# DefTruth/CUDA-Learn-Notes

Measured on NVIDIA H100. Metric: hgemm_tflops, higher is better.
Workload: dtype f16 (fp32 accumulate)

## Files before the change

### cuda-learn-notes_b200/csrc/hgemm_wgmma.cu

```cuda
#include "abi_common.cuh"
#include "ptx.cuh"

namespace b200k {

namespace gemm {
constexpr int BM = 128, BN = 256, STAGES = 4, THREADS = 384, GROUP_M = 16;
constexpr int STG_BYTES = 16384;
}

template <int DT_, bool A_MN_, bool B_MN_>
struct GemmCfg {
  static constexpr int DT = DT_;
  static constexpr bool A_MN = A_MN_, B_MN = B_MN_;
  static constexpr int ES = DT == 2 ? 4 : 2;
  static constexpr int BK = 128 / ES;
  static constexpr int KSTEP = DT == 2 ? 8 : 16;
  static constexpr int A_BYTES = gemm::BM * BK * ES;
  static constexpr int B_BYTES = gemm::BN * BK * ES;
  static constexpr int STAGE_BYTES = A_BYTES + B_BYTES;
  static constexpr int SMEM_BYTES = gemm::STAGES * STAGE_BYTES + 2 * gemm::STG_BYTES + 1024 + 2 * gemm::STAGES * 8;
  static_assert(!(DT == 2 && (A_MN || B_MN)), "tf32 wgmma reads K-major operands only");
  static_assert(SMEM_BYTES <= 232448, "more shared memory than an H100 block may use");
};

template <class Cfg>
__device__ __forceinline__ void gemm_mma_kblock(float* d, uint32_t sA, uint32_t sB, int cw) {
  constexpr int STEPS = Cfg::BK / Cfg::KSTEP;
#pragma unroll
  for (int k = 0; k < STEPS; ++k) {
    const uint64_t da = Cfg::A_MN ? wgmma_desc(sA + cw * 64 * Cfg::BK * Cfg::ES + k * 2048, 64 * Cfg::BK * Cfg::ES, 1024)
                                  : wgmma_desc(sA + cw * 64 * 128 + k * 32, 16, 1024);
    const uint64_t db = Cfg::B_MN ? wgmma_desc(sB + k * 2048, 64 * Cfg::BK * Cfg::ES, 1024) : wgmma_desc(sB + k * 32, 16, 1024);
    wgmma_ss<Cfg::DT, 256, Cfg::A_MN, Cfg::B_MN>(d, da, db, 1);
  }
}

template <class Cfg>
__device__ __forceinline__ void gemm_store_tile(const float* d, const CUtensorMap* tmC, uint32_t stg, int cw, int row0,
                                                int col0) {
  constexpr int SLICES = Cfg::DT == 2 ? 4 : 2, JS = 32 / SLICES, JB = JS / 2;
  const int t = threadIdx.x & 127, lane = t & 31, warp = t / 32;
  const bool leader = t == 0;
#pragma unroll
  for (int sl = 0; sl < SLICES; ++sl) {
    if (leader) tma_store_wait_read<0>();
    named_bar_sync(1 + cw, 128);
    if constexpr (Cfg::DT == 2) {
      const int q = lane & 3;
#pragma unroll
      for (int jj = 0; jj < JS; ++jj) {
        const int j = sl * JS + jj;
#pragma unroll
        for (int h = 0; h < 2; ++h) {
          const int r = warp * 16 + 8 * h + lane / 4;
          const int chunk = 2 * (jj % JB) + q / 2;
          const uint32_t a = stg + (jj / JB) * 8192 + r * 128 + ((chunk ^ (r & 7)) << 4) + (q & 1) * 8;
          asm volatile("st.shared.v2.f32 [%0], {%1, %2};" ::"r"(a), "f"(d[4 * j + 2 * h]), "f"(d[4 * j + 2 * h + 1])
                       : "memory");
        }
      }
    } else {
      const int m = lane / 8, r = warp * 16 + 8 * (m & 1) + (lane & 7);
#pragma unroll
      for (int jj = 0; jj < JS; jj += 2) {
        const int j = sl * JS + jj, chunk = jj % JB + (m >> 1);
        const uint32_t a = stg + (jj / JB) * 8192 + r * 128 + ((chunk ^ (r & 7)) << 4);
        uint32_t p[4];
#pragma unroll
        for (int i = 0; i < 4; ++i)
          p[i] = Cfg::DT == 1 ? pack_bf162(d[4 * j + 2 * i], d[4 * j + 2 * i + 1])
                              : pack_half2(d[4 * j + 2 * i], d[4 * j + 2 * i + 1]);
        stmatrix_x4(a, p[0], p[1], p[2], p[3]);
      }
    }
    fence_proxy_async_smem();
    named_bar_sync(1 + cw, 128);
    if (leader) {
      const int c = col0 + sl * (gemm::BN / SLICES);
      tma_store_2d(tmC, stg, c, row0);
      tma_store_2d(tmC, stg + 8192, c + 128 / Cfg::ES, row0);
      tma_store_commit();
    }
  }
}

template <class Cfg>
__global__ void __launch_bounds__(gemm::THREADS, 1)
    hgemm_wgmma_kernel(const __grid_constant__ CUtensorMap tmA, const __grid_constant__ CUtensorMap tmB,
                       const __grid_constant__ CUtensorMap tmC, int K, int tiles_m, int tiles_n) {
  using namespace gemm;
  extern __shared__ uint8_t smem_raw[];
  const uint32_t base = (smem_u32(smem_raw) + 1023) & ~1023u;
  const uint32_t stg0 = base + STAGES * Cfg::STAGE_BYTES;
  const uint32_t full0 = stg0 + 2 * STG_BYTES, empty0 = full0 + STAGES * 8;
  const int wg = threadIdx.x / 128;

  const int tile = blockIdx.x, width = GROUP_M * tiles_n, g = tile / width, first_m = g * GROUP_M;
  const int gsz = min(tiles_m - first_m, GROUP_M);
  const int tm = first_m + (tile % width) % gsz, tn = (tile % width) / gsz;
  const int nkb = (K + Cfg::BK - 1) / Cfg::BK;

  if (threadIdx.x == 0) {
    for (int s = 0; s < STAGES; ++s) {
      mbar_init(full0 + 8 * s, 1);
      mbar_init(empty0 + 8 * s, 2);
    }
    fence_mbar_init();
  }
  __syncthreads();

  if (wg == 0) {
    if (threadIdx.x == 0) {
      tma_prefetch_desc(&tmA);
      tma_prefetch_desc(&tmB);
      for (int kb = 0; kb < nkb; ++kb) {
        const int s = kb % STAGES;
        if (kb >= STAGES) mbar_wait_nocall(empty0 + 8 * s, ((kb / STAGES) - 1) & 1);
        const uint32_t bar = full0 + 8 * s, sA = base + s * Cfg::STAGE_BYTES, sB = sA + Cfg::A_BYTES;
        mbar_arrive_expect_tx(bar, Cfg::STAGE_BYTES);
        if constexpr (Cfg::A_MN) {
#pragma unroll
          for (int c = 0; c < BM / 64; ++c)
            tma_load_2d(sA + c * 64 * Cfg::BK * Cfg::ES, &tmA, bar, tm * BM + c * 64, kb * Cfg::BK, kPolicyEvictNormal);
        } else {
          tma_load_2d(sA, &tmA, bar, kb * Cfg::BK, tm * BM, kPolicyEvictNormal);
        }
        if constexpr (Cfg::B_MN) {
#pragma unroll
          for (int c = 0; c < BN / 64; ++c)
            tma_load_2d(sB + c * 64 * Cfg::BK * Cfg::ES, &tmB, bar, tn * BN + c * 64, kb * Cfg::BK, kPolicyEvictNormal);
        } else {
          tma_load_2d(sB, &tmB, bar, kb * Cfg::BK, tn * BN, kPolicyEvictNormal);
        }
      }
    }
    return;
  }

  const int cw = wg - 1, t = threadIdx.x & 127;
  const bool leader = t == 0;
  if (leader) tma_prefetch_desc(&tmC);
  float d[128];
#pragma unroll
  for (int i = 0; i < 128; ++i) d[i] = 0.f;
  for (int kb = 0; kb < nkb; ++kb) {
    const int s = kb % STAGES;
    mbar_wait_nocall(full0 + 8 * s, (kb / STAGES) & 1);
    const uint32_t sA = base + s * Cfg::STAGE_BYTES, sB = sA + Cfg::A_BYTES;
    fence_regs<128>(d);
    wgmma_fence();
    gemm_mma_kblock<Cfg>(d, sA, sB, cw);
    wgmma_commit();
    wgmma_wait<1>();
    fence_regs<128>(d);
    if (kb > 0 && leader) mbar_arrive(empty0 + 8 * ((kb - 1) % STAGES));
  }
  wgmma_wait<0>();
  fence_regs<128>(d);
  gemm_store_tile<Cfg>(d, &tmC, stg0 + cw * STG_BYTES, cw, tm * BM + cw * 64, tn * BN);
  if (leader) tma_store_wait_all<0>();
}

template <class Cfg>
static int launch_gemm(const void* A, const void* B, void* C, int64_t M, int64_t N, int64_t K, cudaStream_t s,
                       const DeviceInfo& di) {
  using namespace gemm;
  auto tmap = [](CUtensorMap* m, const void* p, int64_t rows, int64_t cols, uint32_t box_rows, uint32_t box_cols) {
    const uint64_t dims[2] = {uint64_t(cols), uint64_t(rows)}, strides[1] = {uint64_t(cols) * Cfg::ES};
    const uint32_t box[2] = {box_cols, box_rows};
    return make_tmap(m, p, Cfg::ES, 2, dims, strides, box);
  };
  CUtensorMap tmA, tmB, tmC;
  int rc = Cfg::A_MN ? tmap(&tmA, A, K, M, Cfg::BK, 64) : tmap(&tmA, A, M, K, BM, Cfg::BK);
  if (rc) return rc;
  rc = Cfg::B_MN ? tmap(&tmB, B, K, N, Cfg::BK, 64) : tmap(&tmB, B, N, K, BN, Cfg::BK);
  if (rc) return rc;
  if ((rc = tmap(&tmC, C, M, N, 64, 128 / Cfg::ES))) return rc;
  const int64_t tiles_m = (M + BM - 1) / BM, tiles_n = (N + BN - 1) / BN, tiles = tiles_m * tiles_n;
  if (tiles > INT32_MAX) return set_error(B200K_ESHAPE, "GEMM too large: %lld tiles", (long long)tiles);
  auto kern = hgemm_wgmma_kernel<Cfg>;
  if ((rc = ensure_dynamic_smem(reinterpret_cast<const void*>(kern), di.device, Cfg::SMEM_BYTES))) return rc;
  kern<<<unsigned(tiles), THREADS, Cfg::SMEM_BYTES, s>>>(tmA, tmB, tmC, int(K), int(tiles_m), int(tiles_n));
  B200K_CHECK_CUDA(cudaGetLastError());
  return B200K_OK;
}

template <int DT>
static int gemm_dispatch(const char* who, const void* A, const void* B, void* C, int64_t M, int64_t N, int64_t K,
                         int b_is_nk, int variant, void* stream, int a_is_km = 0) {
  constexpr int PACK = (DT == 2) ? 4 : 8;
  if (!A || !B || !C) return set_error(B200K_EARG, "%s: null pointer", who);
  if (reinterpret_cast<uintptr_t>(C) & 15) return set_error(B200K_EALIGN, "%s: C (%p) must be 16-byte aligned", who, C);
  if (M < 1 || N < 1 || K < 1 || M > INT32_MAX || N > INT32_MAX || K > INT32_MAX)
    return set_error(B200K_ESHAPE, "%s: M,N,K must be in [1, 2^31) (got %lld,%lld,%lld)", who, (long long)M, (long long)N,
                     (long long)K);
  if ((K % PACK) || (N % PACK))
    return set_error(B200K_ESHAPE, "%s: K and N must be multiples of %d (16-byte rows), got K=%lld N=%lld", who, PACK,
                     (long long)K, (long long)N);
  if (a_is_km && DT == 2) return set_error(B200K_EDTYPE, "%s: A stored as [K,M] is built for f16 / bf16 only", who);
  if (a_is_km && (M % PACK))
    return set_error(B200K_ESHAPE, "%s: M must be a multiple of %d when A is stored as [K,M]", who, PACK);
  const int v = variant & 0xff;
  if (v < B200K_HGEMM_AUTO || v > B200K_HGEMM_2CTA_512x256)
    return set_error(B200K_EARG, "%s: variant %d unknown", who, v);
  DeviceInfo di;
  int rc = get_device_info(&di);
  if (rc) return rc;
  cudaStream_t s = static_cast<cudaStream_t>(stream);
  const bool nn = (b_is_nk == 0);
  if constexpr (DT == 2) {
    if (!nn) return launch_gemm<GemmCfg<2, false, false>>(A, B, C, M, N, K, s, di);
    void* bt = nullptr;
    B200K_CHECK_CUDA(cudaMallocAsync(&bt, size_t(K) * size_t(N) * 4, s));
    rc = b200k_mat_transpose_f32(B, bt, K, N, stream);
    if (!rc) rc = launch_gemm<GemmCfg<2, false, false>>(A, bt, C, M, N, K, s, di);
    cudaError_t e = cudaFreeAsync(bt, s);
    if (!rc && e != cudaSuccess) rc = set_error(B200K_ECUDA, "cudaFreeAsync failed: %s", cudaGetErrorString(e));
    return rc;
  } else {
    if (a_is_km)
      return nn ? launch_gemm<GemmCfg<DT, true, true>>(A, B, C, M, N, K, s, di)
                : launch_gemm<GemmCfg<DT, true, false>>(A, B, C, M, N, K, s, di);
    return nn ? launch_gemm<GemmCfg<DT, false, true>>(A, B, C, M, N, K, s, di)
              : launch_gemm<GemmCfg<DT, false, false>>(A, B, C, M, N, K, s, di);
  }
}

}

extern "C" int b200k_hgemm_f16(const void* A, const void* B, void* C, int64_t M, int64_t N, int64_t K, int b_is_nk,
                               int variant, void* stream) {
  return b200k::gemm_dispatch<0>("b200k_hgemm_f16", A, B, C, M, N, K, b_is_nk, variant, stream);
}

extern "C" int b200k_gemm_ex(const void* A, const void* B, void* C, int64_t M, int64_t N, int64_t K, int a_is_km, int b_is_nk,
                             int dtype, int variant, void* stream) {
  switch (dtype) {
    case B200K_F16: return b200k::gemm_dispatch<0>("b200k_gemm_ex(f16)", A, B, C, M, N, K, b_is_nk, variant, stream, a_is_km);
    case B200K_BF16: return b200k::gemm_dispatch<1>("b200k_gemm_ex(bf16)", A, B, C, M, N, K, b_is_nk, variant, stream, a_is_km);
    case B200K_F32: return b200k::gemm_dispatch<2>("b200k_gemm_ex(tf32)", A, B, C, M, N, K, b_is_nk, variant, stream, a_is_km);
    default: return b200k::set_error(B200K_EDTYPE, "b200k_gemm_ex: dtype %d not supported (f16, bf16, f32-as-tf32)", dtype);
  }
}

extern "C" int b200k_gemm(const void* A, const void* B, void* C, int64_t M, int64_t N, int64_t K, int b_is_nk, int dtype,
                          int variant, void* stream) {
  switch (dtype) {
    case B200K_F16: return b200k::gemm_dispatch<0>("b200k_gemm(f16)", A, B, C, M, N, K, b_is_nk, variant, stream);
    case B200K_BF16: return b200k::gemm_dispatch<1>("b200k_gemm(bf16)", A, B, C, M, N, K, b_is_nk, variant, stream);
    case B200K_F32: return b200k::gemm_dispatch<2>("b200k_gemm(tf32)", A, B, C, M, N, K, b_is_nk, variant, stream);
    default: return b200k::set_error(B200K_EDTYPE, "b200k_gemm: dtype %d not supported (f16, bf16, f32-as-tf32)", dtype);
  }
}
```

### cuda-learn-notes_b200/csrc/ptx.cuh

```cuda
#pragma once
#include <cstdint>
#include <cuda.h>
#include <cuda_bf16.h>
#include <cuda_fp16.h>
#include <cuda_runtime.h>

namespace b200k {

#ifndef B200K_SPIN_LIMIT_CYCLES
#define B200K_SPIN_LIMIT_CYCLES (10LL * 1000 * 1000 * 1000)
#endif

__device__ __forceinline__ uint32_t smem_u32(const void* p) {
  return static_cast<uint32_t>(__cvta_generic_to_shared(p));
}
__device__ __forceinline__ void named_bar_sync(uint32_t id, uint32_t nthreads) {
  asm volatile("bar.sync %0, %1;" ::"r"(id), "r"(nthreads) : "memory");
}

__device__ __forceinline__ void mbar_init(uint32_t bar, uint32_t count) {
  asm volatile("mbarrier.init.shared::cta.b64 [%0], %1;" ::"r"(bar), "r"(count) : "memory");
}
__device__ __forceinline__ void fence_mbar_init() {
  asm volatile("fence.mbarrier_init.release.cluster;" ::: "memory");
}
__device__ __forceinline__ void fence_proxy_async_smem() {
  asm volatile("fence.proxy.async.shared::cta;" ::: "memory");
}
__device__ __forceinline__ void mbar_arrive(uint32_t bar) {
  asm volatile("mbarrier.arrive.shared::cta.b64 _, [%0];" ::"r"(bar) : "memory");
}
__device__ __forceinline__ void mbar_arrive_expect_tx(uint32_t bar, uint32_t bytes) {
  asm volatile("mbarrier.arrive.expect_tx.shared::cta.b64 _, [%0], %1;" ::"r"(bar), "r"(bytes) : "memory");
}
__device__ __forceinline__ uint32_t mbar_try_wait(uint32_t bar, uint32_t parity) {
  uint32_t ok;
  asm volatile(
      "{\n\t"
      ".reg .pred P1;\n\t"
      "mbarrier.try_wait.parity.shared::cta.b64 P1, [%1], %2;\n\t"
      "selp.u32 %0, 1, 0, P1;\n\t"
      "}"
      : "=r"(ok)
      : "r"(bar), "r"(parity)
      : "memory");
  return ok;
}
static __device__ __noinline__ void mbar_timeout_trap(uint32_t bar, uint32_t parity) {
  printf("[b200k] mbarrier wait timed out: block (%d,%d) thread %d bar 0x%x parity %u\n", blockIdx.x, blockIdx.y,
         threadIdx.x, bar, parity);
  __trap();
}
__device__ __forceinline__ void mbar_wait(uint32_t bar, uint32_t parity) {
  if (mbar_try_wait(bar, parity)) return;
  long long t0 = clock64();
  while (!mbar_try_wait(bar, parity)) {
    if (clock64() - t0 > B200K_SPIN_LIMIT_CYCLES) mbar_timeout_trap(bar, parity);
  }
}
__device__ __forceinline__ void mbar_wait_nocall(uint32_t bar, uint32_t parity) {
  if (mbar_try_wait(bar, parity)) return;
  long long t0 = clock64();
  while (!mbar_try_wait(bar, parity)) {
    if (clock64() - t0 > B200K_SPIN_LIMIT_CYCLES) asm volatile("trap;");
  }
}

__device__ __forceinline__ void tma_prefetch_desc(const CUtensorMap* m) {
  asm volatile("prefetch.tensormap [%0];" ::"l"(reinterpret_cast<uint64_t>(m)) : "memory");
}
constexpr uint64_t kPolicyEvictNormal = 0x1000000000000000ull;
constexpr uint64_t kPolicyEvictFirst = 0x12F0000000000000ull;

__device__ __forceinline__ void tma_load_2d(uint32_t dst_smem, const CUtensorMap* m, uint32_t bar, int32_t c0,
                                            int32_t c1, uint64_t policy) {
  asm volatile(
      "cp.async.bulk.tensor.2d.shared::cluster.global.mbarrier::complete_tx::bytes.L2::cache_hint"
      " [%0], [%1, {%3, %4}], [%2], %5;" ::"r"(dst_smem),
      "l"(reinterpret_cast<uint64_t>(m)), "r"(bar), "r"(c0), "r"(c1), "l"(policy)
      : "memory");
}
__device__ __forceinline__ void tma_load_3d(uint32_t dst_smem, const CUtensorMap* m, uint32_t bar, int32_t c0,
                                            int32_t c1, int32_t c2, uint64_t policy) {
  asm volatile(
      "cp.async.bulk.tensor.3d.shared::cluster.global.mbarrier::complete_tx::bytes.L2::cache_hint"
      " [%0], [%1, {%3, %4, %5}], [%2], %6;" ::"r"(dst_smem),
      "l"(reinterpret_cast<uint64_t>(m)), "r"(bar), "r"(c0), "r"(c1), "r"(c2), "l"(policy)
      : "memory");
}
__device__ __forceinline__ void tma_store_2d(const CUtensorMap* m, uint32_t src_smem, int32_t c0, int32_t c1) {
  asm volatile("cp.async.bulk.tensor.2d.global.shared::cta.bulk_group [%0, {%2, %3}], [%1];" ::"l"(
                   reinterpret_cast<uint64_t>(m)),
               "r"(src_smem), "r"(c0), "r"(c1)
               : "memory");
}
__device__ __forceinline__ void tma_store_commit() { asm volatile("cp.async.bulk.commit_group;" ::: "memory"); }
template <int N>
__device__ __forceinline__ void tma_store_wait_read() {
  asm volatile("cp.async.bulk.wait_group.read %0;" ::"n"(N) : "memory");
}
template <int N>
__device__ __forceinline__ void tma_store_wait_all() {
  asm volatile("cp.async.bulk.wait_group %0;" ::"n"(N) : "memory");
}
__device__ __forceinline__ void stmatrix_x4(uint32_t addr, uint32_t r0, uint32_t r1, uint32_t r2, uint32_t r3) {
  asm volatile("stmatrix.sync.aligned.m8n8.x4.shared.b16 [%0], {%1, %2, %3, %4};" ::"r"(addr), "r"(r0), "r"(r1), "r"(r2),
               "r"(r3)
               : "memory");
}

__device__ __forceinline__ uint64_t wgmma_desc(uint32_t smem_addr, uint32_t lbo, uint32_t sbo) {
  return uint64_t((smem_addr & 0x3FFFF) >> 4) | (uint64_t(lbo >> 4) << 16) | (uint64_t(sbo >> 4) << 32) | (1ull << 62);
}
__device__ __forceinline__ void wgmma_fence() { asm volatile("wgmma.fence.sync.aligned;" ::: "memory"); }
__device__ __forceinline__ void wgmma_commit() { asm volatile("wgmma.commit_group.sync.aligned;" ::: "memory"); }
template <int N>
__device__ __forceinline__ void wgmma_wait() { asm volatile("wgmma.wait_group.sync.aligned %0;" ::"n"(N) : "memory"); }
template <int N>
__device__ __forceinline__ void fence_regs(float* d) {
#pragma unroll
  for (int i = 0; i < N; ++i) asm volatile("" : "+f"(d[i])::"memory");
}

#define B200K_ACC8(i) \
  "+f"(d[i]), "+f"(d[i + 1]), "+f"(d[i + 2]), "+f"(d[i + 3]), "+f"(d[i + 4]), "+f"(d[i + 5]), "+f"(d[i + 6]), "+f"(d[i + 7])
#define B200K_ACC32(i) B200K_ACC8(i), B200K_ACC8(i + 8), B200K_ACC8(i + 16), B200K_ACC8(i + 24)
#define B200K_ACC64 B200K_ACC32(0)
#define B200K_ACC128 B200K_ACC64, B200K_ACC32(32)
#define B200K_ACC192 B200K_ACC128, B200K_ACC32(64)
#define B200K_ACC256 B200K_ACC192, B200K_ACC32(96)
#define B200K_PH64 \
  "%0, %1, %2, %3, %4, %5, %6, %7, %8, %9, %10, %11, %12, %13, %14, %15, " \
  "%16, %17, %18, %19, %20, %21, %22, %23, %24, %25, %26, %27, %28, %29, %30, %31"
#define B200K_PH128 \
  B200K_PH64 ", %32, %33, %34, %35, %36, %37, %38, %39, %40, %41, %42, %43, %44, %45, %46, %47, " \
  "%48, %49, %50, %51, %52, %53, %54, %55, %56, %57, %58, %59, %60, %61, %62, %63"
#define B200K_PH192 \
  B200K_PH128 ", %64, %65, %66, %67, %68, %69, %70, %71, %72, %73, %74, %75, %76, %77, %78, %79, " \
  "%80, %81, %82, %83, %84, %85, %86, %87, %88, %89, %90, %91, %92, %93, %94, %95"
#define B200K_PH256 \
  B200K_PH192 ", %96, %97, %98, %99, %100, %101, %102, %103, %104, %105, %106, %107, %108, %109, %110, %111, " \
  "%112, %113, %114, %115, %116, %117, %118, %119, %120, %121, %122, %123, %124, %125, %126, %127"
#define B200K_WGMMA(shape, type, acc, scale, ops) \
  "{\n.reg .pred p;\nsetp.ne.b32 p, " scale ", 0;\n" \
  "wgmma.mma_async.sync.aligned." shape ".f32." type " {" acc "}, " ops ";\n}\n"
#define B200K_SS(type, n, scale, ops) \
  asm volatile(B200K_WGMMA("m64n" #n "k16", type, B200K_PH##n, scale, ops) \
               : B200K_ACC##n \
               : "l"(da), "l"(db), "r"(scale_d), "n"(TA), "n"(TB))
#define B200K_RS(type, n, scale, ops) \
  asm volatile(B200K_WGMMA("m64n" #n "k16", type, B200K_PH##n, scale, ops) \
               : B200K_ACC##n \
               : "r"(a[0]), "r"(a[1]), "r"(a[2]), "r"(a[3]), "l"(db), "r"(scale_d), "n"(TB))
#define B200K_F16_OR_BF16(op, ...) \
  if constexpr (DT == 0) \
    op("f16.f16", __VA_ARGS__); \
  else \
    op("bf16.bf16", __VA_ARGS__)

template <int DT, int N, int TA, int TB>
__device__ __forceinline__ void wgmma_ss(float* d, uint64_t da, uint64_t db, int scale_d) {
  static_assert(N == 64 || N == 128 || N == 256, "wgmma_ss: N must be 64, 128 or 256");
  static_assert(DT == 0 || DT == 1 || (DT == 2 && N == 256 && TA == 0 && TB == 0),
                "wgmma_ss: f16 / bf16, or tf32 with N = 256 and K-major operands");
  if constexpr (DT == 2) {
    asm volatile(B200K_WGMMA("m64n256k8", "tf32.tf32", B200K_PH256, "%130", "%128, %129, p, 1, 1")
                 : B200K_ACC256
                 : "l"(da), "l"(db), "r"(scale_d));
  } else if constexpr (N == 64) {
    B200K_F16_OR_BF16(B200K_SS, 64, "%34", "%32, %33, p, 1, 1, %35, %36");
  } else if constexpr (N == 128) {
    B200K_F16_OR_BF16(B200K_SS, 128, "%66", "%64, %65, p, 1, 1, %67, %68");
  } else {
    B200K_F16_OR_BF16(B200K_SS, 256, "%130", "%128, %129, p, 1, 1, %131, %132");
  }
}
template <int DT, int N, int TB>
__device__ __forceinline__ void wgmma_rs(float* d, const uint32_t* a, uint64_t db, int scale_d) {
  static_assert(N == 64 || N == 128 || N == 192 || N == 256, "wgmma_rs: N must be 64, 128, 192 or 256");
  static_assert(DT == 0 || DT == 1, "wgmma_rs: f16 or bf16");
  if constexpr (N == 64) {
    B200K_F16_OR_BF16(B200K_RS, 64, "%37", "{%32, %33, %34, %35}, %36, p, 1, 1, %38");
  } else if constexpr (N == 128) {
    B200K_F16_OR_BF16(B200K_RS, 128, "%69", "{%64, %65, %66, %67}, %68, p, 1, 1, %70");
  } else if constexpr (N == 192) {
    B200K_F16_OR_BF16(B200K_RS, 192, "%101", "{%96, %97, %98, %99}, %100, p, 1, 1, %102");
  } else {
    B200K_F16_OR_BF16(B200K_RS, 256, "%133", "{%128, %129, %130, %131}, %132, p, 1, 1, %134");
  }
}
#undef B200K_ACC8
#undef B200K_ACC32
#undef B200K_ACC64
#undef B200K_ACC128
#undef B200K_ACC192
#undef B200K_ACC256
#undef B200K_PH64
#undef B200K_PH128
#undef B200K_PH192
#undef B200K_PH256
#undef B200K_WGMMA
#undef B200K_SS
#undef B200K_RS
#undef B200K_F16_OR_BF16

__device__ __forceinline__ uint32_t pack_half2(float lo, float hi) {
  __half2 h = __floats2half2_rn(lo, hi);
  return *reinterpret_cast<uint32_t*>(&h);
}
__device__ __forceinline__ uint32_t pack_bf162(float lo, float hi) {
  __nv_bfloat162 h = __floats2bfloat162_rn(lo, hi);
  return *reinterpret_cast<uint32_t*>(&h);
}

}
```

Before: 767.3.

## Multicast B tiles across 2-CTA clusters with cross-CTA empty barriers

Launches the GEMM kernel as clusters of two CTAs that share the same N tile. Each CTA loads half of the B tile and multicasts it to both CTAs, roughly halving B traffic from L2. To keep this safe, each CTA's empty barriers now count arrivals from both CTAs' consumers, and cluster barriers replace __syncthreads at start and exit. It rounds tiles_m up to an even count, which can launch extra out-of-bounds tiles, and couples the pipeline progress of the two paired CTAs.

```diff
diff --git a/cuda-learn-notes_b200/csrc/hgemm_wgmma.cu b/cuda-learn-notes_b200/csrc/hgemm_wgmma.cu
--- a/cuda-learn-notes_b200/csrc/hgemm_wgmma.cu
+++ b/cuda-learn-notes_b200/csrc/hgemm_wgmma.cu
@@ -85,7 +85,7 @@
 }
 
 template <class Cfg>
-__global__ void __launch_bounds__(gemm::THREADS, 1)
+__global__ void __cluster_dims__(2, 1, 1) __launch_bounds__(gemm::THREADS, 1)
     hgemm_wgmma_kernel(const __grid_constant__ CUtensorMap tmA, const __grid_constant__ CUtensorMap tmB,
                        const __grid_constant__ CUtensorMap tmC, int K, int tiles_m, int tiles_n) {
   using namespace gemm;
@@ -94,6 +94,7 @@
   const uint32_t stg0 = base + STAGES * Cfg::STAGE_BYTES;
   const uint32_t full0 = stg0 + 2 * STG_BYTES, empty0 = full0 + STAGES * 8;
   const int wg = threadIdx.x / 128;
+  const uint32_t rank = cluster_ctarank();
 
   const int tile = blockIdx.x, width = GROUP_M * tiles_n, g = tile / width, first_m = g * GROUP_M;
   const int gsz = min(tiles_m - first_m, GROUP_M);
@@ -103,11 +104,13 @@
   if (threadIdx.x == 0) {
     for (int s = 0; s < STAGES; ++s) {
       mbar_init(full0 + 8 * s, 1);
-      mbar_init(empty0 + 8 * s, 2);
+      mbar_init(empty0 + 8 * s, 4);
     }
     fence_mbar_init();
   }
-  __syncthreads();
+  __syncwarp();
+  cluster_arrive();
+  cluster_wait();
 
   if (wg == 0) {
     if (threadIdx.x == 0) {
@@ -127,38 +130,49 @@
         }
         if constexpr (Cfg::B_MN) {
 #pragma unroll
-          for (int c = 0; c < BN / 64; ++c)
-            tma_load_2d(sB + c * 64 * Cfg::BK * Cfg::ES, &tmB, bar, tn * BN + c * 64, kb * Cfg::BK, kPolicyEvictNormal);
+          for (int c = 2 * rank; c < 2 * rank + 2; ++c)
+            tma_load_2d_multicast(sB + c * 64 * Cfg::BK * Cfg::ES, &tmB, bar, tn * BN + c * 64, kb * Cfg::BK, 0b11,
+                                  kPolicyEvictNormal);
         } else {
-          tma_load_2d(sB, &tmB, bar, kb * Cfg::BK, tn * BN, kPolicyEvictNormal);
+          tma_load_2d_multicast(sB + rank * (BN / 2) * 128, &tmB, bar, kb * Cfg::BK, tn * BN + rank * (BN / 2), 0b11,
+                                kPolicyEvictNormal);
         }
       }
     }
-    return;
-  }
-
-  const int cw = wg - 1, t = threadIdx.x & 127;
-  const bool leader = t == 0;
-  if (leader) tma_prefetch_desc(&tmC);
-  float d[128];
-#pragma unroll
-  for (int i = 0; i < 128; ++i) d[i] = 0.f;
-  for (int kb = 0; kb < nkb; ++kb) {
-    const int s = kb % STAGES;
-    mbar_wait_nocall(full0 + 8 * s, (kb / STAGES) & 1);
-    const uint32_t sA = base + s * Cfg::STAGE_BYTES, sB = sA + Cfg::A_BYTES;
+    __syncwarp();
+    cluster_arrive();
+  } else {
+    const int cw = wg - 1, t = threadIdx.x & 127;
+    const bool leader = t == 0;
+    if (leader) tma_prefetch_desc(&tmC);
+    float d[128];
+#pragma unroll
+    for (int i = 0; i < 128; ++i) d[i] = 0.f;
+    for (int kb = 0; kb < nkb; ++kb) {
+      const int s = kb % STAGES;
+      mbar_wait_nocall(full0 + 8 * s, (kb / STAGES) & 1);
+      const uint32_t sA = base + s * Cfg::STAGE_BYTES, sB = sA + Cfg::A_BYTES;
+      fence_regs<128>(d);
+      wgmma_fence();
+      gemm_mma_kblock<Cfg>(d, sA, sB, cw);
+      wgmma_commit();
+      wgmma_wait<1>();
+      fence_regs<128>(d);
+      if (kb > 0 && leader) {
+        const uint32_t bar = empty0 + 8 * ((kb - 1) % STAGES);
+        mbar_arrive_cluster(mapa(bar, 0));
+        mbar_arrive_cluster(mapa(bar, 1));
+      }
+    }
+    __syncwarp();
+    cluster_arrive();
+    wgmma_wait<0>();
     fence_regs<128>(d);
-    wgmma_fence();
-    gemm_mma_kblock<Cfg>(d, sA, sB, cw);
-    wgmma_commit();
-    wgmma_wait<1>();
-    fence_regs<128>(d);
-    if (kb > 0 && leader) mbar_arrive(empty0 + 8 * ((kb - 1) % STAGES));
-  }
-  wgmma_wait<0>();
-  fence_regs<128>(d);
-  gemm_store_tile<Cfg>(d, &tmC, stg0 + cw * STG_BYTES, cw, tm * BM + cw * 64, tn * BN);
-  if (leader) tma_store_wait_all<0>();
+    gemm_store_tile<Cfg>(d, &tmC, stg0 + cw * STG_BYTES, cw, tm * BM + cw * 64, tn * BN);
+    if (leader) tma_store_wait_all<0>();
+  }
+  __syncwarp();
+  cluster_wait();
 }
 
 template <class Cfg>
@@ -173,10 +187,10 @@
   CUtensorMap tmA, tmB, tmC;
   int rc = Cfg::A_MN ? tmap(&tmA, A, K, M, Cfg::BK, 64) : tmap(&tmA, A, M, K, BM, Cfg::BK);
   if (rc) return rc;
-  rc = Cfg::B_MN ? tmap(&tmB, B, K, N, Cfg::BK, 64) : tmap(&tmB, B, N, K, BN, Cfg::BK);
+  rc = Cfg::B_MN ? tmap(&tmB, B, K, N, Cfg::BK, 64) : tmap(&tmB, B, N, K, BN / 2, Cfg::BK);
   if (rc) return rc;
   if ((rc = tmap(&tmC, C, M, N, 64, 128 / Cfg::ES))) return rc;
-  const int64_t tiles_m = (M + BM - 1) / BM, tiles_n = (N + BN - 1) / BN, tiles = tiles_m * tiles_n;
+  const int64_t tiles_m = (M + 2 * BM - 1) / (2 * BM) * 2, tiles_n = (N + BN - 1) / BN, tiles = tiles_m * tiles_n;
   if (tiles > INT32_MAX) return set_error(B200K_ESHAPE, "GEMM too large: %lld tiles", (long long)tiles);
   auto kern = hgemm_wgmma_kernel<Cfg>;
   if ((rc = ensure_dynamic_smem(reinterpret_cast<const void*>(kern), di.device, Cfg::SMEM_BYTES))) return rc;
diff --git a/cuda-learn-notes_b200/csrc/ptx.cuh b/cuda-learn-notes_b200/csrc/ptx.cuh
--- a/cuda-learn-notes_b200/csrc/ptx.cuh
+++ b/cuda-learn-notes_b200/csrc/ptx.cuh
@@ -18,6 +18,23 @@
   asm volatile("bar.sync %0, %1;" ::"r"(id), "r"(nthreads) : "memory");
 }
 
+__device__ __forceinline__ uint32_t cluster_ctarank() {
+  uint32_t r;
+  asm volatile("mov.u32 %0, %%cluster_ctarank;" : "=r"(r));
+  return r;
+}
+__device__ __forceinline__ uint32_t mapa(uint32_t local_smem_addr, uint32_t rank) {
+  uint32_t r;
+  asm volatile("mapa.shared::cluster.u32 %0, %1, %2;" : "=r"(r) : "r"(local_smem_addr), "r"(rank));
+  return r;
+}
+__device__ __forceinline__ void cluster_arrive() {
+  asm volatile("barrier.cluster.arrive.release.aligned;" ::: "memory");
+}
+__device__ __forceinline__ void cluster_wait() {
+  asm volatile("barrier.cluster.wait.acquire.aligned;" ::: "memory");
+}
+
 __device__ __forceinline__ void mbar_init(uint32_t bar, uint32_t count) {
   asm volatile("mbarrier.init.shared::cta.b64 [%0], %1;" ::"r"(bar), "r"(count) : "memory");
 }
@@ -29,6 +46,9 @@
 }
 __device__ __forceinline__ void mbar_arrive(uint32_t bar) {
   asm volatile("mbarrier.arrive.shared::cta.b64 _, [%0];" ::"r"(bar) : "memory");
+}
+__device__ __forceinline__ void mbar_arrive_cluster(uint32_t cluster_bar) {
+  asm volatile("mbarrier.arrive.shared::cluster.b64 _, [%0];" ::"r"(cluster_bar) : "memory");
 }
 __device__ __forceinline__ void mbar_arrive_expect_tx(uint32_t bar, uint32_t bytes) {
   asm volatile("mbarrier.arrive.expect_tx.shared::cta.b64 _, [%0], %1;" ::"r"(bar), "r"(bytes) : "memory");
@@ -78,6 +98,14 @@
       "cp.async.bulk.tensor.2d.shared::cluster.global.mbarrier::complete_tx::bytes.L2::cache_hint"
       " [%0], [%1, {%3, %4}], [%2], %5;" ::"r"(dst_smem),
       "l"(reinterpret_cast<uint64_t>(m)), "r"(bar), "r"(c0), "r"(c1), "l"(policy)
+      : "memory");
+}
+__device__ __forceinline__ void tma_load_2d_multicast(uint32_t dst_smem, const CUtensorMap* m, uint32_t bar, int32_t c0,
+                                                      int32_t c1, uint16_t cta_mask, uint64_t policy) {
+  asm volatile(
+      "cp.async.bulk.tensor.2d.shared::cluster.global.mbarrier::complete_tx::bytes.multicast::cluster.L2::cache_hint"
+      " [%0], [%1, {%3, %4}], [%2], %5, %6;" ::"r"(dst_smem),
+      "l"(reinterpret_cast<uint64_t>(m)), "r"(bar), "r"(c0), "r"(c1), "h"(cta_mask), "l"(policy)
       : "memory");
 }
 __device__ __forceinline__ void tma_load_3d(uint32_t dst_smem, const CUtensorMap* m, uint32_t bar, int32_t c0,
```

New measurement: 763.7 (median of 6 runs). No clear change (-0.5%).
